# SchlomoFeng/GDN

Measured on AMD Instinct MI355X. Metric: sliding-windows/sec forward+anomaly-score, SWaT-shape (127 sensors, W=15), higher is better.
Workload: dtype f32; 1 GPU; BASELINE configs[2]: SWaT-shape eval forward + anomaly score; sensors=127, window=15, topk=30, dim=64, out_layer_num=1, batch=512, batches_per_launch=64, windows_per_launch=32768, storage=fp32, multi_gpu_measured=False, hip_graph=True, forward_streams=3, parallelism=single GPU

## Files before the change

### gdn_amd/csrc/gdn_score.hip

```cpp
#pragma clang fp contract(off)
#include "gdn_common.hpp"

#include <stdlib.h>

namespace {

constexpr int NQ = 6;

struct SelectArgs {
  int rank[NQ];
  double gamma[2];
  int median_pair;
};

constexpr unsigned long long FILLER = ~0ull;

__global__ __launch_bounds__(256) void score_keys_kernel(const float* __restrict__ pred,
                                                         const float* __restrict__ gt, int t, int n, int pitch,
                                                         double* __restrict__ keys) {
  __shared__ double tile[64][65];
  const int t0 = blockIdx.x * 64, s0 = blockIdx.y * 64;
  const int lane = threadIdx.x & 63, wv = threadIdx.x >> 6;
  for (int r = wv; r < 64; r += 4) {
    const int tick = t0 + r, s = s0 + lane;
    if (tick < t && s < n) {
      const size_t o = (size_t)tick * n + s;
      tile[r][lane] = fabs((double)pred[o] - (double)gt[o]);
    }
  }
  __syncthreads();
  for (int r = wv; r < 64; r += 4) {
    const int s = s0 + r, tick = t0 + lane;
    if (s < n && tick < pitch)
      keys[(size_t)s * pitch + tick] = tick < t ? tile[lane][r] : __longlong_as_double((long long)FILLER);
  }
}

constexpr int SLICE = 2048;

struct SelState {
  unsigned long long prefix[NQ];
  int rem[NQ];
  int rep[NQ];
  unsigned int hist[NQ][256];
  unsigned int arrive;
  unsigned int cnt_b;
  unsigned int digits_done;
  unsigned int pad1;
};

struct KeyLayout {
  const unsigned long long* keys;
  unsigned long long* bufb;
  int blocks, n, pitch;
};

__global__ void select_init_kernel(SelState* __restrict__ state, const SelectArgs sa) {
  SelState& st = state[blockIdx.x];
  for (int i = threadIdx.x; i < NQ * 256; i += blockDim.x) (&st.hist[0][0])[i] = 0u;
  if (threadIdx.x < NQ) {
    st.prefix[threadIdx.x] = 0ull;
    st.rem[threadIdx.x] = sa.rank[threadIdx.x];
    st.rep[threadIdx.x] = 0;
  }
  if (threadIdx.x == 0) {
    st.arrive = 0u;
    st.cnt_b = 0u;
    st.digits_done = 0u;
  }
}

__device__ __forceinline__ void locate_bin(const unsigned int* h, int left0, unsigned long long pf, int shift,
                                           int lane, unsigned long long* npf, int* nrem) {
  const uint4 c4 = *reinterpret_cast<const uint4*>(h + 4 * lane);
  const int mine = (int)(c4.x + c4.y + c4.z + c4.w);
  int incl = mine;
#pragma unroll
  for (int d = 1; d < 64; d <<= 1) {
    const int up = __shfl_up(incl, d);
    if (lane >= d) incl += up;
  }
  const int excl = incl - mine;
  if (left0 >= excl && left0 < incl) {
    int left = left0 - excl, bin = 0;
    const int c[4] = {(int)c4.x, (int)c4.y, (int)c4.z, (int)c4.w};
#pragma unroll
    for (int j = 0; j < 3; ++j) {
      if (bin == j && left >= c[j]) {
        left -= c[j];
        bin = j + 1;
      }
    }
    *npf = pf | ((unsigned long long)(4 * lane + bin) << shift);
    *nrem = left;
  }
}

__device__ __forceinline__ void write_result(const unsigned long long* prefix, const SelectArgs& sa, int s,
                                             double* __restrict__ med_iqr) {
  double v[NQ];
  for (int q = 0; q < NQ; ++q) v[q] = __longlong_as_double((long long)prefix[q]);
  const double med = sa.median_pair ? (v[0] + v[1]) / 2.0 : v[0];
  double qv[2];
  for (int h = 0; h < 2; ++h) {
    const double a = v[2 + 2 * h], b = v[3 + 2 * h], gm = sa.gamma[h];
    const double diff = b - a;
    double r = a + diff * gm;
    if (gm >= 0.5) r = b - diff * (1.0 - gm);
    qv[h] = r;
  }
  med_iqr[2 * s] = med;
  med_iqr[2 * s + 1] = qv[1] - qv[0];
}

template <bool FROM_B, bool COMPACT>
__global__ __launch_bounds__(256) void select_pass_kernel(const KeyLayout kl, SelState* __restrict__ state,
                                                          int pass) {
  __shared__ unsigned int hist[NQ][256];
  __shared__ unsigned long long stage[COMPACT ? SLICE : 1];
  __shared__ unsigned int n_stage, out_base, ticket_s;
  __shared__ unsigned long long npf[NQ];
  __shared__ int nrem[NQ];
  const int s = blockIdx.y, g = blockIdx.x, G = gridDim.x;
  const int tid = threadIdx.x, lane = tid & 63, wv = tid >> 6;
  SelState& st = state[s];
  if (!FROM_B && !COMPACT && pass == 1 && st.digits_done >= 2u) return;
  const unsigned int slots = (unsigned int)kl.blocks * (unsigned int)kl.pitch;
  const unsigned int cnt = FROM_B ? st.cnt_b : slots;
  unsigned long long* outb = kl.bufb + (size_t)s * slots;
  const int shift = 56 - 8 * pass;
  const bool two = !FROM_B && !COMPACT && pass == 0;
  const unsigned int dref = two ? (unsigned int)(kl.keys[(size_t)s * kl.pitch] >> 56) : 0u;
  unsigned long long pf[NQ];
  bool active[NQ];
#pragma unroll
  for (int q = 0; q < NQ; ++q) {
    pf[q] = st.prefix[q];
    active[q] = st.rep[q] == q;
  }
  for (int i = tid; i < NQ * 256; i += 256) (&hist[0][0])[i] = 0u;
  if (tid == 0) n_stage = 0u;
  __syncthreads();

  for (unsigned int base = (unsigned int)g * SLICE; base < cnt; base += (unsigned int)G * SLICE) {
    const unsigned long long* in;
    unsigned int lim;
    if (FROM_B) {
      in = outb + base;
      lim = cnt - base;
    } else {
      const unsigned int blk = base / (unsigned int)kl.pitch, off = base - blk * (unsigned int)kl.pitch;
      in = kl.keys + ((size_t)blk * kl.n + s) * kl.pitch + off;
      lim = (unsigned int)kl.pitch - off;
    }
    unsigned long long key[8];
#pragma unroll
    for (int u = 0; u < 8; ++u) {
      const unsigned int i = tid + u * 256;
      key[u] = i < lim ? in[i] : FILLER;
    }
#pragma unroll
    for (int u = 0; u < 8; ++u) {
      const bool real = key[u] != FILLER;
      const unsigned int digit = (unsigned int)(key[u] >> shift) & 255u;
      const unsigned int d0 = __builtin_amdgcn_readfirstlane(digit);
      bool any = false;
#pragma unroll
      for (int q = 0; q < NQ; ++q) {
        if (!active[q]) continue;
        const bool match = real && (pass == 0 ? true : ((key[u] ^ pf[q]) >> (shift + 8)) == 0ull);
        any |= match;
        if (__all(match && digit == d0)) {
          if (lane == 0) atomicAdd(&hist[q][d0], 64u);
        } else if (match) {
          atomicAdd(&hist[q][digit], 1u);
        }
      }
      if constexpr (COMPACT) {
        if (any) stage[atomicAdd(&n_stage, 1u)] = key[u];
      }
      if (two && real && digit == dref) atomicAdd(&hist[1][(unsigned int)(key[u] >> 48) & 255u], 1u);
    }
    if constexpr (COMPACT) {
      __syncthreads();
      if (tid == 0) out_base = n_stage ? atomicAdd(&st.cnt_b, n_stage) : 0u;
      __syncthreads();
      for (unsigned int i = tid; i < n_stage; i += 256) outb[out_base + i] = stage[i];
      __syncthreads();
      if (tid == 0) n_stage = 0u;
      __syncthreads();
    }
  }
  __syncthreads();
  for (int i = tid; i < NQ * 256; i += 256) {
    const unsigned int c = (&hist[0][0])[i];
    if (c) atomicAdd(&(&st.hist[0][0])[i], c);
  }
  asm volatile("s_waitcnt vmcnt(0)" ::: "memory");
  __syncthreads();
  if (tid == 0) ticket_s = atomicAdd(&st.arrive, 1u);
  __syncthreads();
  if (ticket_s != (unsigned int)(G - 1)) return;

  for (int i = tid; i < NQ * 256; i += 256) (&hist[0][0])[i] = atomicExch(&(&st.hist[0][0])[i], 0u);
  __syncthreads();
  for (int q = wv; q < NQ; q += 4) locate_bin(hist[st.rep[q]], st.rem[q], pf[q], shift, lane, &npf[q], &nrem[q]);
  __syncthreads();
  unsigned int done = (unsigned int)pass + 1u;
  if (two) {
    bool inside = dref != 255u;
    for (int q = 0; q < NQ; ++q) inside = inside && (unsigned int)(npf[q] >> 56) == dref;
    if (inside) {
      __shared__ unsigned long long npf2[NQ];
      __shared__ int nrem2[NQ];
      for (int q = wv; q < NQ; q += 4) locate_bin(hist[1], nrem[q], npf[q], shift - 8, lane, &npf2[q], &nrem2[q]);
      __syncthreads();
      if (tid < NQ) {
        npf[tid] = npf2[tid];
        nrem[tid] = nrem2[tid];
      }
      __syncthreads();
      done = 2u;
    }
  }
  if (tid < NQ) {
    st.prefix[tid] = npf[tid];
    st.rem[tid] = nrem[tid];
    int r = tid;
    for (int q = tid - 1; q >= 0; --q)
      if (npf[q] == npf[tid]) r = q;
    st.rep[tid] = r;
  }
  if (tid == 0) {
    st.digits_done = done;
    atomicExch(&st.arrive, 0u);
  }
}

constexpr int FIN_NT = 1024;
template <bool FROM_B>
__global__ __launch_bounds__(FIN_NT) void select_finish_kernel(const KeyLayout kl, SelState* __restrict__ state,
                                                            int first_pass, const SelectArgs sa,
                                                            double* __restrict__ med_iqr) {
  __shared__ unsigned int hist[NQ][256];
  __shared__ unsigned long long prefix[NQ];
  __shared__ int rem[NQ];
  __shared__ int rep[NQ];
  const int s = blockIdx.x;
  const int tid = threadIdx.x, lane = tid & 63, wv = tid >> 6;
  SelState& st = state[s];
  const unsigned int slots = (unsigned int)kl.blocks * (unsigned int)kl.pitch;
  const unsigned int cnt = FROM_B ? st.cnt_b : slots;
  const unsigned long long* in = FROM_B ? kl.bufb + (size_t)s * slots : kl.keys + (size_t)s * kl.pitch;
  if (tid < NQ) {
    prefix[tid] = st.prefix[tid];
    rem[tid] = st.rem[tid];
  }
  constexpr int FK = 32;
  const bool resident = cnt <= FK * FIN_NT;
  unsigned long long key[FK];
  if (resident) {
#pragma unroll
    for (int u = 0; u < FK; ++u) {
      const unsigned int i = tid + u * FIN_NT;
      key[u] = i < cnt ? in[i] : FILLER;
    }
  }
  __syncthreads();
  for (int pass = first_pass; pass < 8; ++pass) {
    const int shift = 56 - 8 * pass;
    if (tid < NQ) {
      int r = tid;
      for (int q = tid - 1; q >= 0; --q)
        if (prefix[q] == prefix[tid]) r = q;
      rep[tid] = r;
    }
    for (int i = tid; i < NQ * 256; i += FIN_NT) (&hist[0][0])[i] = 0u;
    __syncthreads();
    unsigned long long pf[NQ];
    bool active[NQ];
#pragma unroll
    for (int q = 0; q < NQ; ++q) {
      pf[q] = prefix[q];
      active[q] = rep[q] == q;
    }
    auto tally = [&](unsigned long long k) -> bool {
      if (k == FILLER) return false;
      const unsigned int digit = (unsigned int)(k >> shift) & 255u;
      bool any = false;
#pragma unroll
      for (int q = 0; q < NQ; ++q) {
        if (!active[q]) continue;
        if (pass == 0 || ((k ^ pf[q]) >> (shift + 8)) == 0ull) {
          atomicAdd(&hist[q][digit], 1u);
          any = true;
        }
      }
      return any;
    };
    if (resident) {
#pragma unroll
      for (int u = 0; u < FK; ++u)
        if (!tally(key[u])) key[u] = FILLER;
    } else {
      for (unsigned int i = tid; i < cnt; i += FIN_NT) tally(in[i]);
    }
    __syncthreads();
    for (int q = wv; q < NQ; q += FIN_NT / 64) locate_bin(hist[rep[q]], rem[q], pf[q], shift, lane, &prefix[q], &rem[q]);
    __syncthreads();
  }
  if (tid == 0) write_result(prefix, sa, s, med_iqr);
}

constexpr int ONE_NT = 1024;
constexpr int ONE_FK = 32;
constexpr int ONE_CAP = 8192;
constexpr int ONE_CAP2 = 1024;

template <bool FLAT>
__global__ __launch_bounds__(ONE_NT) void select_onewg_kernel(const KeyLayout kl, const SelectArgs sa,
                                                              double* __restrict__ med_iqr) {
  __shared__ unsigned int hist[NQ][256];
  __shared__ unsigned long long prefix[NQ];
  __shared__ unsigned long long stage[ONE_CAP];
  __shared__ unsigned long long stage2[ONE_CAP2];
  __shared__ unsigned short sidx[ONE_CAP];
  __shared__ int rem[NQ];
  __shared__ int rep[NQ];
  __shared__ unsigned int n_stage, n_stage2, dref;
  __shared__ unsigned int cnt0[2];
  const int s = blockIdx.x;
  const int tid = threadIdx.x, lane = tid & 63, wv = tid >> 6;
  const unsigned int slots = (unsigned int)kl.blocks * (unsigned int)kl.pitch;
#ifdef GDN_SELECT_TIMING
  const long long tick_start = wall_clock64();
#endif
  constexpr bool flat = FLAT;
  const __amdgpu_buffer_rsrc_t rsrc = __builtin_amdgcn_make_buffer_rsrc(
      const_cast<unsigned long long*>(kl.keys + (size_t)s * kl.pitch), 0, flat ? kl.pitch * 8 : 0, 0x00020000);
  auto key_full = [&](int u) -> unsigned long long {
    if constexpr (flat) {
      typedef unsigned int u32x2 __attribute__((ext_vector_type(2)));
      const u32x2 v = __builtin_amdgcn_raw_buffer_load_b64(rsrc, tid * 8, u * (ONE_NT * 8), 0);
      return ((unsigned long long)v.y << 32) | v.x;
    } else {
      const unsigned int i = tid + u * ONE_NT;
      const unsigned int blk = i / (unsigned int)kl.pitch, off = i - blk * (unsigned int)kl.pitch;
      return kl.keys[((size_t)blk * kl.n + s) * kl.pitch + off];
    }
  };
  auto key_slot = [&](unsigned int i) -> unsigned long long {
    if constexpr (flat) {
      return kl.keys[(size_t)s * kl.pitch + i];
    } else {
      const unsigned int blk = i / (unsigned int)kl.pitch, off = i - blk * (unsigned int)kl.pitch;
      return kl.keys[((size_t)blk * kl.n + s) * kl.pitch + off];
    }
  };
  unsigned int khi[ONE_FK];
#pragma unroll
  for (int u = 0; u < ONE_FK; ++u) {
    unsigned int hi;
    if constexpr (flat) hi = __builtin_amdgcn_raw_buffer_load_b32(rsrc, tid * 8 + 4, u * (ONE_NT * 8), 0);
    else hi = tid + u * ONE_NT < slots ? (unsigned int)(key_full(u) >> 32) : 0u;
    khi[u] = tid + u * ONE_NT < slots ? hi : 0xffffffffu;
  }
  if (tid < NQ) {
    prefix[tid] = 0ull;
    rem[tid] = sa.rank[tid];
  }
  if (tid == 0) {
    n_stage = 0u;
    n_stage2 = 0u;
  }
  __syncthreads();
#ifdef GDN_SELECT_TIMING
  long long tick[12];
  int nt = 0;
  tick[nt++] = wall_clock64();
#endif
  bool in_lds = false;
  bool done = false;
  unsigned int n_keep = 0u;
  for (int pass = 0; pass < 8 && !done; ++pass) {
    const int shift = 56 - 8 * pass;
    if (tid < NQ) {
      int r = tid;
      for (int q = tid - 1; q >= 0; --q)
        if (prefix[q] == prefix[tid]) r = q;
      rep[tid] = r;
    }
    for (int i = tid; i < NQ * 256; i += ONE_NT) (&hist[0][0])[i] = 0u;
    if (pass == 0 && tid == 0) {
      cnt0[0] = cnt0[1] = 0u;
      dref = khi[0] >> 24;
    }
    __syncthreads();
    if (pass == 0) {
      const unsigned int dr = dref;
      unsigned int less = 0u, same = 0u;
#pragma unroll
      for (int u = 0; u < ONE_FK; ++u) {
        const unsigned int hi = khi[u];
        const unsigned int digit = hi >> 24;
        less += digit < dr ? 1u : 0u;
        same += digit == dr ? 1u : 0u;
      }
#pragma unroll
      for (int d = 32; d >= 1; d >>= 1) {
        less += __shfl_xor(less, d);
        same += __shfl_xor(same, d);
      }
      if (lane == 0) {
        atomicAdd(&cnt0[0], less);
        atomicAdd(&cnt0[1], same);
      }
      __syncthreads();
      const unsigned int tl = cnt0[0], ts = cnt0[1];
      bool inside = dr != 255u;
#pragma unroll
      for (int q = 0; q < NQ; ++q) inside = inside && (unsigned int)sa.rank[q] >= tl && (unsigned int)sa.rank[q] < tl + ts;
      if (inside) {
        if (tid < NQ) {
          prefix[tid] = (unsigned long long)dr << 56;
          rem[tid] = sa.rank[tid] - (int)tl;
        }
        __syncthreads();
#ifdef GDN_SELECT_TIMING
        tick[nt++] = wall_clock64();
#endif
        continue;
      }
    }
    if (!in_lds && pass < 3) {
      const unsigned int sh = 24u - 8u * (unsigned int)pass;
#pragma nounroll
      for (int q = 0; q < NQ; ++q) {
        if (rep[q] != q) continue;
        const unsigned int pfh = (unsigned int)(prefix[q] >> 32);
        unsigned int* hq = hist[q];
#pragma unroll
        for (int u = 0; u < ONE_FK; ++u) {
          const unsigned int hi = khi[u];
          const bool real = (int)hi >= 0;
          const unsigned int digit = (hi >> sh) & 255u;
          if (pass == 0) {
            const unsigned int d0 = __builtin_amdgcn_readfirstlane(digit);
            if (__all(real && digit == d0)) {
              if (lane == 0) atomicAdd(&hq[d0], 64u);
            } else if (real) {
              atomicAdd(&hq[digit], 1u);
            }
          } else if (real && ((hi ^ pfh) >> (sh + 8u)) == 0u) {
            atomicAdd(&hq[digit], 1u);
          }
        }
      }
    } else if (!in_lds) {
#pragma nounroll
      for (int q = 0; q < NQ; ++q) {
        if (rep[q] != q) continue;
        const unsigned long long pfq = prefix[q];
        unsigned int* hq = hist[q];
#pragma unroll 4
        for (int u = 0; u < ONE_FK; ++u) {
          const bool real = (int)khi[u] >= 0;
          const unsigned long long k = real ? key_full(u) : FILLER;
          const unsigned int digit = (unsigned int)(k >> shift) & 255u;
          if (real && ((k ^ pfq) >> (shift + 8)) == 0ull) atomicAdd(&hq[digit], 1u);
        }
      }
    } else {
#pragma nounroll
      for (int q = 0; q < NQ; ++q) {
        if (rep[q] != q) continue;
        const unsigned long long pfq = prefix[q];
        unsigned int* hq = hist[q];
        for (unsigned int i = tid; i < n_keep; i += ONE_NT) {
          const unsigned long long k = stage[i];
          const unsigned int digit = (unsigned int)(k >> shift) & 255u;
          if (((k ^ pfq) >> (shift + 8)) == 0ull) atomicAdd(&hq[digit], 1u);
        }
      }
    }
    __syncthreads();
    for (int q = wv; q < NQ; q += ONE_NT / 64)
      locate_bin(hist[rep[q]], rem[q], prefix[q], shift, lane, &prefix[q], &rem[q]);
    __syncthreads();
    if (pass == 1) {
      unsigned int p16[NQ];
#pragma unroll
      for (int q = 0; q < NQ; ++q) {
        p16[q] = __builtin_amdgcn_readfirstlane((unsigned int)(prefix[q] >> 48));
#pragma unroll
        for (int r = 0; r < q; ++r)
          if (p16[r] == p16[q]) p16[q] = 0x10000u;
      }
      unsigned int keep = 0u;
#pragma unroll
      for (int u = 0; u < ONE_FK; ++u) {
        const unsigned int h16 = khi[u] >> 16;
        bool any = false;
#pragma unroll
        for (int q = 0; q < NQ; ++q) any |= h16 == p16[q];
        keep |= any ? (1u << u) : 0u;
      }
      const int mine = __popc(keep);
      int incl = mine;
#pragma unroll
      for (int d = 1; d < 64; d <<= 1) {
        const int up = __shfl_up(incl, d);
        if (lane >= d) incl += up;
      }
      unsigned int base = 0u;
      if (lane == 63) base = atomicAdd(&n_stage, (unsigned int)incl);
      base = __shfl(base, 63);
      unsigned int pos = base + (unsigned int)(incl - mine);
      unsigned int t1 = tid;
      asm volatile("" : "+v"(t1));
#pragma unroll
      for (int u = 0; u < ONE_FK; ++u) {
        if ((keep >> u) & 1u) {
          if (pos < (unsigned int)ONE_CAP) sidx[pos] = (unsigned short)(t1 + u * ONE_NT);
          ++pos;
        }
      }
      __syncthreads();
      n_keep = n_stage;
      in_lds = n_keep <= (unsigned int)ONE_CAP;
      if (in_lds) {
        for (unsigned int i = tid; i < n_keep; i += ONE_NT) stage[i] = key_slot(sidx[i]);
        __syncthreads();
      }
    }
    if (pass == 2 && in_lds) {
      for (unsigned int i = tid; i < n_keep; i += ONE_NT) {
        const unsigned long long k = stage[i];
        bool any = false;
#pragma unroll
        for (int q = 0; q < NQ; ++q) any |= ((k ^ prefix[q]) >> 40) == 0ull;
        if (any) {
          const unsigned int at = atomicAdd(&n_stage2, 1u);
          if (at < (unsigned int)ONE_CAP2) stage2[at] = k;
        }
      }
      __syncthreads();
      const unsigned int n2 = n_stage2;
      if (n2 <= (unsigned int)ONE_CAP2) {
        if ((unsigned int)tid < n2) {
          const unsigned long long k = stage2[tid];
#pragma unroll
          for (int q = 0; q < NQ; ++q) {
            const unsigned long long pq = prefix[q];
            if (((k ^ pq) >> 40) != 0ull) continue;
            int less = 0, equal = 0;
            for (unsigned int j = 0; j < n2; ++j) {
              const unsigned long long o = stage2[j];
              if (((o ^ pq) >> 40) != 0ull) continue;
              less += o < k ? 1 : 0;
              equal += o == k ? 1 : 0;
            }
            const int want = rem[q];
            if (less <= want && want < less + equal) prefix[q] = k;
          }
        }
        __syncthreads();
        done = true;
      }
    }
#ifdef GDN_SELECT_TIMING
    tick[nt++] = wall_clock64();
#endif
  }
#ifdef GDN_SELECT_TIMING
  if (tid == 0 && s == 1)
    printf("onewg ticks(10ns): load %lld p0 %lld p1+compact %lld p2+finish %lld (passes run %d) survivors %u / %u\n",
           tick[0] - tick_start, tick[1] - tick[0], tick[2] - tick[1], tick[3] - tick[2], nt - 1, n_keep, n_stage2);
#endif
  if (tid == 0) write_result(prefix, sa, s, med_iqr);
}

constexpr int RUN = 8;

__global__ __launch_bounds__(256) void score_smooth_max_kernel(
    const float* __restrict__ pred, const float* __restrict__ gt, const double* __restrict__ med_iqr,
    int t, int n, int first_tick, const float* __restrict__ halo_pred, const float* __restrict__ halo_gt,
    double* __restrict__ scores, double* __restrict__ anomaly) {
  __shared__ double best[4][RUN];
  const int lane = threadIdx.x & 63, wv = threadIdx.x >> 6;
  const int wpb = blockDim.x >> 6;
  const int nruns = (t + RUN - 1) / RUN;
  for (int run = blockIdx.x * wpb + wv; run < nruns; run += gridDim.x * wpb) {
    const int t0 = run * RUN, t1 = min(t, t0 + RUN);
    for (int s0 = 0; s0 < n; s0 += 128) {
      const int sa_ = s0 + lane, sb_ = s0 + 64 + lane;
      const bool la = sa_ < n, lb = sb_ < n;
      const int ca = la ? sa_ : n - 1, cb = lb ? sb_ : n - 1;
      const double meda = med_iqr[2 * ca], dena = 1.0 / (fabs(med_iqr[2 * ca + 1]) + 1e-2);
      const double medb = med_iqr[2 * cb], denb = 1.0 / (fabs(med_iqr[2 * cb + 1]) + 1e-2);
      const int g0 = first_tick + t0;
      float pa[RUN + 3], ga[RUN + 3], pb[RUN + 3], gb[RUN + 3];
#pragma unroll
      for (int u = 0; u < RUN + 3; ++u) {
        const int tt = t0 - 3 + u;
        const bool halo = tt < 0;
        const int row = halo ? (first_tick > 0 ? 3 + tt : 0) : min(tt, t - 1);
        const float* pp = (halo && first_tick > 0 ? halo_pred : pred) + (size_t)row * n;
        const float* gg = (halo && first_tick > 0 ? halo_gt : gt) + (size_t)row * n;
        pa[u] = pp[ca]; ga[u] = gg[ca]; pb[u] = pp[cb]; gb[u] = gg[cb];
      }
      auto norm = [&](float pv, float gv, double med, double inv_den) -> double {
        return (fabs((double)pv - (double)gv) - med) * inv_den;
      };
      double a3 = g0 >= 3 ? norm(pa[0], ga[0], meda, dena) : 0.0;
      double a2 = g0 >= 2 ? norm(pa[1], ga[1], meda, dena) : 0.0;
      double a1 = g0 >= 1 ? norm(pa[2], ga[2], meda, dena) : 0.0;
      double b3 = g0 >= 3 ? norm(pb[0], gb[0], medb, denb) : 0.0;
      double b2 = g0 >= 2 ? norm(pb[1], gb[1], medb, denb) : 0.0;
      double b1 = g0 >= 1 ? norm(pb[2], gb[2], medb, denb) : 0.0;
      double mt[RUN];
#pragma unroll
      for (int u = 0; u < RUN; ++u) {
        const int tick = t0 + u;
        mt[u] = -INFINITY;
        if (tick < t1) {
          const double a0 = norm(pa[3 + u], ga[3 + u], meda, dena);
          const double b0 = norm(pb[3 + u], gb[3 + u], medb, denb);
          double sma = 0.0, smb = 0.0;
          if (first_tick + tick >= 3) {
            sma = (((a3 + a2) + a1) + a0) / 4.0;
            smb = (((b3 + b2) + b1) + b0) / 4.0;
          }
          if (scores) {
            if (la) scores[(size_t)sa_ * t + tick] = sma;
            if (lb) scores[(size_t)sb_ * t + tick] = smb;
          }
          mt[u] = fmax(la ? sma : -INFINITY, lb ? smb : -INFINITY);
          a3 = a2; a2 = a1; a1 = a0;
          b3 = b2; b2 = b1; b1 = b0;
        }
      }
      static_assert(RUN == 8, "the transposing reduction is written for 8 ticks");
      double k4[4], k2[2], k1;
      {
        const bool up = (lane & 32) != 0;
#pragma unroll
        for (int i2 = 0; i2 < 4; ++i2) {
          const double mine = up ? mt[4 + i2] : mt[i2], send = up ? mt[i2] : mt[4 + i2];
          k4[i2] = fmax(mine, __shfl_xor(send, 32));
        }
      }
      {
        const bool up = (lane & 16) != 0;
#pragma unroll
        for (int i2 = 0; i2 < 2; ++i2) {
          const double mine = up ? k4[2 + i2] : k4[i2], send = up ? k4[i2] : k4[2 + i2];
          k2[i2] = fmax(mine, __shfl_xor(send, 16));
        }
      }
      {
        const bool up = (lane & 8) != 0;
        const double mine = up ? k2[1] : k2[0], send = up ? k2[0] : k2[1];
        k1 = fmax(mine, __shfl_xor(send, 8));
      }
      k1 = fmax(k1, __shfl_xor(k1, 4));
      k1 = fmax(k1, __shfl_xor(k1, 2));
      k1 = fmax(k1, __shfl_xor(k1, 1));
      if ((lane & 7) == 0) {
        const int u = ((lane >> 5) & 1) * 4 + ((lane >> 4) & 1) * 2 + ((lane >> 3) & 1);
        best[wv][u] = s0 == 0 ? k1 : fmax(best[wv][u], k1);
      }
    }
    if (lane < t1 - t0) anomaly[t0 + lane] = best[wv][lane];
  }
}

}

namespace {

SelectArgs make_select_args(long long t) {
  SelectArgs sa;
  sa.median_pair = (t % 2 == 0);
  sa.rank[0] = (int)(sa.median_pair ? t / 2 - 1 : (t - 1) / 2);
  sa.rank[1] = (int)(sa.median_pair ? t / 2 : (t - 1) / 2);
  const double qs[2] = {25.0 / 100.0, 75.0 / 100.0};
  for (int h = 0; h < 2; ++h) {
    const double vi = (double)t * qs[h] + (1.0 + qs[h] * (1.0 - 1.0 - 1.0)) - 1.0;
    const double lo = floor(vi);
    long long ilo = (long long)lo, ihi = ilo + 1;
    if (ilo < 0) ilo = 0;
    if (ihi > t - 1) ihi = t - 1;
    if (ilo > t - 1) ilo = t - 1;
    sa.rank[2 + 2 * h] = (int)ilo;
    sa.rank[3 + 2 * h] = (int)ihi;
    sa.gamma[h] = vi - lo;
  }
  return sa;
}

bool force_multi_block() {
  static int v = -1;
  if (v < 0) {
    const char* e = getenv("GDN_SELECT_MULTI");
    v = (e && e[0] == '1') ? 1 : 0;
  }
  return v == 1;
}

int run_select(const double* keys, int blocks, int n, int pitch, long long total, double* workspace,
               double* med_iqr, hipStream_t st) {
  const long long slots = (long long)blocks * pitch;
  KeyLayout kl;
  kl.keys = reinterpret_cast<const unsigned long long*>(keys);
  kl.bufb = reinterpret_cast<unsigned long long*>(workspace);
  kl.blocks = blocks; kl.n = n; kl.pitch = pitch;
  SelState* state = reinterpret_cast<SelState*>(kl.bufb + (size_t)slots * n);
  const SelectArgs sa = make_select_args(total);
  const int slices = (int)((slots + SLICE - 1) / SLICE);
  if (slices > 1 && slots <= (long long)ONE_NT * ONE_FK && !force_multi_block()) {
    if (kl.blocks == 1) hipLaunchKernelGGL(select_onewg_kernel<true>, dim3(n), dim3(ONE_NT), 0, st, kl, sa, med_iqr);
    else hipLaunchKernelGGL(select_onewg_kernel<false>, dim3(n), dim3(ONE_NT), 0, st, kl, sa, med_iqr);
    return gdn_launch_status();
  }
  hipLaunchKernelGGL(select_init_kernel, dim3(n), dim3(256), 0, st, state, sa);
  if (slices == 1) {
    hipLaunchKernelGGL(select_finish_kernel<false>, dim3(n), dim3(FIN_NT), 0, st, kl, state, 0, sa, med_iqr);
    return gdn_launch_status();
  }
  hipLaunchKernelGGL((select_pass_kernel<false, false>), dim3(slices, n), dim3(256), 0, st, kl, state, 0);
  hipLaunchKernelGGL((select_pass_kernel<false, false>), dim3(slices, n), dim3(256), 0, st, kl, state, 1);
  hipLaunchKernelGGL((select_pass_kernel<false, true>), dim3(slices, n), dim3(256), 0, st, kl, state, 2);
  hipLaunchKernelGGL(select_finish_kernel<true>, dim3(n), dim3(FIN_NT), 0, st, kl, state, 3, sa, med_iqr);
  return gdn_launch_status();
}

}

extern "C" long long gdn_score_select_workspace_bytes(int blocks, int n, int pitch) {
  if (blocks <= 0 || n <= 0 || pitch <= 0) return 0;
  return (long long)blocks * pitch * n * 8 + (long long)n * (long long)sizeof(SelState) + 256;
}

extern "C" long long gdn_score_workspace_bytes(int t, int n) {
  if (t <= 0 || n <= 0) return 0;
  return (long long)t * n * 8 + gdn_score_select_workspace_bytes(1, n, t);
}

extern "C" int gdn_score_keys(const float* pred, const float* gt, int t, int n, int pitch, double* keys,
                              void* stream) {
  if (!pred || !gt || !keys || t <= 0 || n <= 0 || pitch < t) return GDN_ERR_ARG;
  hipLaunchKernelGGL(score_keys_kernel, dim3((pitch + 63) / 64, (n + 63) / 64), dim3(256), 0,
                     (hipStream_t)stream, pred, gt, t, n, pitch, keys);
  return gdn_launch_status();
}

extern "C" int gdn_score_select(const double* keys, int blocks, int n, int pitch, long long total,
                                double* workspace, double* med_iqr, void* stream) {
  if (!keys || !workspace || !med_iqr || blocks <= 0 || n <= 0 || pitch <= 0 || total <= 0) return GDN_ERR_ARG;
  if (total > (long long)blocks * pitch || (long long)blocks * pitch > 0x7fffffffll) return GDN_ERR_ARG;
  if (blocks > 1 && pitch % SLICE != 0) return GDN_ERR_UNSUPPORTED;
  return run_select(keys, blocks, n, pitch, total, workspace, med_iqr, (hipStream_t)stream);
}

extern "C" int gdn_score_quantiles(const float* pred, const float* gt, int t, int n, double* workspace,
                                   double* med_iqr, void* stream) {
  if (!pred || !gt || !workspace || !med_iqr || t <= 0 || n <= 0) return GDN_ERR_ARG;
  double* keys = workspace;
  const int rc = gdn_score_keys(pred, gt, t, n, t, keys, stream);
  if (rc != GDN_OK) return rc;
  return run_select(keys, 1, n, t, t, workspace + (size_t)t * n, med_iqr, (hipStream_t)stream);
}

extern "C" int gdn_score_smooth_max(const float* pred, const float* gt, const double* med_iqr, int t, int n,
                                    int first_tick, const float* halo_pred, const float* halo_gt,
                                    double* scores, double* anomaly, void* stream) {
  if (!pred || !gt || !med_iqr || !anomaly || t <= 0 || n <= 0 || first_tick < 0) return GDN_ERR_ARG;
  if (first_tick > 0 && (!halo_pred || !halo_gt)) return GDN_ERR_ARG;
  const int runs = (t + RUN - 1) / RUN;
  const int grid = min((runs + 3) / 4, gdn_cu_count() * 8);
  hipLaunchKernelGGL(score_smooth_max_kernel, dim3(grid), dim3(256), 0, (hipStream_t)stream, pred, gt,
                     med_iqr, t, n, first_tick, halo_pred, halo_gt, scores, anomaly);
  return gdn_launch_status();
}
```

Baseline: 137.7 million windows/s.

## Select quantiles from a compact 32-bit high-word plane, recomputing low bits on demand

```diff
diff --git a/gdn_amd/csrc/gdn_score.hip b/gdn_amd/csrc/gdn_score.hip
--- a/gdn_amd/csrc/gdn_score.hip
+++ b/gdn_amd/csrc/gdn_score.hip
@@ -14,25 +14,31 @@
 };
 
 constexpr unsigned long long FILLER = ~0ull;
-
+constexpr unsigned int FILLER_HI = ~0u;
+
+__device__ __forceinline__ unsigned long long score_key(const float* __restrict__ pred, const float* __restrict__ gt,
+                                                        size_t o) {
+  return (unsigned long long)__double_as_longlong(fabs((double)pred[o] - (double)gt[o]));
+}
+
+template <typename K>
 __global__ __launch_bounds__(256) void score_keys_kernel(const float* __restrict__ pred,
                                                          const float* __restrict__ gt, int t, int n, int pitch,
-                                                         double* __restrict__ keys) {
-  __shared__ double tile[64][65];
+                                                         K* __restrict__ keys) {
+  __shared__ K tile[64][65];
   const int t0 = blockIdx.x * 64, s0 = blockIdx.y * 64;
   const int lane = threadIdx.x & 63, wv = threadIdx.x >> 6;
   for (int r = wv; r < 64; r += 4) {
     const int tick = t0 + r, s = s0 + lane;
     if (tick < t && s < n) {
-      const size_t o = (size_t)tick * n + s;
-      tile[r][lane] = fabs((double)pred[o] - (double)gt[o]);
+      const unsigned long long key = score_key(pred, gt, (size_t)tick * n + s);
+      tile[r][lane] = sizeof(K) == 8 ? (K)key : (K)(key >> 32);
     }
   }
   __syncthreads();
   for (int r = wv; r < 64; r += 4) {
     const int s = s0 + r, tick = t0 + lane;
-    if (s < n && tick < pitch)
-      keys[(size_t)s * pitch + tick] = tick < t ? tile[lane][r] : __longlong_as_double((long long)FILLER);
+    if (s < n && tick < pitch) keys[(size_t)s * pitch + tick] = tick < t ? tile[lane][r] : (K)FILLER;
   }
 }
 
@@ -580,6 +586,237 @@
   if (tid == 0) write_result(prefix, sa, s, med_iqr);
 }
 
+constexpr unsigned int NO_PREFIX = 0x80000000u;
+
+__global__ __launch_bounds__(ONE_NT) void select_onewg_hi_kernel(const unsigned int* __restrict__ plane, int pitch,
+                                                                 const float* __restrict__ pred,
+                                                                 const float* __restrict__ gt, int n,
+                                                                 const SelectArgs sa, double* __restrict__ med_iqr) {
+  __shared__ unsigned int hist[NQ][256];
+  __shared__ unsigned long long prefix[NQ];
+  __shared__ unsigned long long cand[ONE_CAP];
+  __shared__ int rem[NQ];
+  __shared__ int rep[NQ];
+  __shared__ unsigned int n_cand, dref;
+  __shared__ unsigned int cnt0[2];
+  const int s = blockIdx.x;
+  const int tid = threadIdx.x, lane = tid & 63, wv = tid >> 6;
+  const unsigned int slots = (unsigned int)pitch;
+#ifdef GDN_SELECT_TIMING
+  const long long tick_start = wall_clock64();
+#endif
+  const __amdgpu_buffer_rsrc_t rsrc = __builtin_amdgcn_make_buffer_rsrc(
+      const_cast<unsigned int*>(plane + (size_t)s * pitch), 0, pitch * 4, 0x00020000);
+  unsigned int khi[ONE_FK];
+#pragma unroll
+  for (int u = 0; u < ONE_FK; ++u) {
+    const unsigned int hi = __builtin_amdgcn_raw_buffer_load_b32(rsrc, tid * 4, u * (ONE_NT * 4), 0);
+    khi[u] = tid + u * ONE_NT < slots ? hi : FILLER_HI;
+  }
+  if (tid < NQ) {
+    prefix[tid] = 0ull;
+    rem[tid] = sa.rank[tid];
+  }
+  if (tid == 0) n_cand = 0u;
+  __syncthreads();
+#ifdef GDN_SELECT_TIMING
+  long long tick[12];
+  int nt = 0;
+  tick[nt++] = wall_clock64();
+#endif
+  bool in_lds = false;
+  unsigned int n_keep = 0u;
+  for (int pass = 0; pass < 8; ++pass) {
+    const int shift = 56 - 8 * pass;
+    if (tid < NQ) {
+      int r = tid;
+      for (int q = tid - 1; q >= 0; --q)
+        if (prefix[q] == prefix[tid]) r = q;
+      rep[tid] = r;
+    }
+    for (int i = tid; i < NQ * 256; i += ONE_NT) (&hist[0][0])[i] = 0u;
+    if (pass == 0 && tid == 0) {
+      cnt0[0] = cnt0[1] = 0u;
+      dref = khi[0] >> 24;
+    }
+    __syncthreads();
+    if (pass == 0) {
+      const unsigned int dr = dref;
+      unsigned int less = 0u, same = 0u;
+#pragma unroll
+      for (int u = 0; u < ONE_FK; ++u) {
+        const unsigned int digit = khi[u] >> 24;
+        less += digit < dr ? 1u : 0u;
+        same += digit == dr ? 1u : 0u;
+      }
+#pragma unroll
+      for (int d = 32; d >= 1; d >>= 1) {
+        less += __shfl_xor(less, d);
+        same += __shfl_xor(same, d);
+      }
+      if (lane == 0) {
+        atomicAdd(&cnt0[0], less);
+        atomicAdd(&cnt0[1], same);
+      }
+      __syncthreads();
+      const unsigned int tl = cnt0[0], ts = cnt0[1];
+      bool inside = dr != 255u;
+#pragma unroll
+      for (int q = 0; q < NQ; ++q) inside = inside && (unsigned int)sa.rank[q] >= tl && (unsigned int)sa.rank[q] < tl + ts;
+      if (inside) {
+        if (tid < NQ) {
+          prefix[tid] = (unsigned long long)dr << 56;
+          rem[tid] = sa.rank[tid] - (int)tl;
+        }
+        __syncthreads();
+#ifdef GDN_SELECT_TIMING
+        tick[nt++] = wall_clock64();
+#endif
+        continue;
+      }
+    }
+    if (pass < 4) {
+      const unsigned int sh = 24u - 8u * (unsigned int)pass;
+#pragma nounroll
+      for (int q = 0; q < NQ; ++q) {
+        if (rep[q] != q) continue;
+        const unsigned int pfh = (unsigned int)(prefix[q] >> 32);
+        unsigned int* hq = hist[q];
+#pragma unroll
+        for (int u = 0; u < ONE_FK; ++u) {
+          const unsigned int hi = khi[u];
+          const bool real = (int)hi >= 0;
+          const unsigned int digit = (hi >> sh) & 255u;
+          if (pass == 0) {
+            const unsigned int d0 = __builtin_amdgcn_readfirstlane(digit);
+            if (__all(real && digit == d0)) {
+              if (lane == 0) atomicAdd(&hq[d0], 64u);
+            } else if (real) {
+              atomicAdd(&hq[digit], 1u);
+            }
+          } else if (real && ((hi ^ pfh) >> (sh + 8u)) == 0u) {
+            atomicAdd(&hq[digit], 1u);
+          }
+        }
+      }
+    } else if (in_lds) {
+#pragma nounroll
+      for (int q = 0; q < NQ; ++q) {
+        if (rep[q] != q) continue;
+        const unsigned long long pfq = prefix[q];
+        unsigned int* hq = hist[q];
+        for (unsigned int i = tid; i < n_keep; i += ONE_NT) {
+          const unsigned long long k = cand[i];
+          const unsigned int digit = (unsigned int)(k >> shift) & 255u;
+          if (((k ^ pfq) >> (shift + 8)) == 0ull) atomicAdd(&hq[digit], 1u);
+        }
+      }
+    } else {
+#pragma nounroll
+      for (int q = 0; q < NQ; ++q) {
+        if (rep[q] != q) continue;
+        const unsigned long long pfq = prefix[q];
+        const unsigned int pfh = (unsigned int)(pfq >> 32);
+        unsigned int* hq = hist[q];
+        unsigned int t1 = tid;
+        asm volatile("" : "+v"(t1));
+#pragma unroll
+        for (int u = 0; u < ONE_FK; ++u) {
+          if (khi[u] != pfh) continue;
+          const unsigned long long k = score_key(pred, gt, (size_t)(t1 + u * ONE_NT) * n + s);
+          const unsigned int digit = (unsigned int)(k >> shift) & 255u;
+          if (((k ^ pfq) >> (shift + 8)) == 0ull) atomicAdd(&hq[digit], 1u);
+        }
+      }
+    }
+    __syncthreads();
+    for (int q = wv; q < NQ; q += ONE_NT / 64)
+      locate_bin(hist[rep[q]], rem[q], prefix[q], shift, lane, &prefix[q], &rem[q]);
+    __syncthreads();
+#ifdef GDN_SELECT_TIMING
+    if (pass < 3) tick[nt++] = wall_clock64();
+#endif
+    if (pass == 3) {
+      unsigned int ph[NQ], p32[NQ];
+#pragma unroll
+      for (int q = 0; q < NQ; ++q) {
+        ph[q] = __builtin_amdgcn_readfirstlane((unsigned int)(prefix[q] >> 32));
+        p32[q] = ph[q];
+#pragma unroll
+        for (int r = 0; r < q; ++r)
+          if (ph[r] == ph[q]) p32[q] = NO_PREFIX;
+      }
+      unsigned int keep = 0u;
+#pragma unroll
+      for (int u = 0; u < ONE_FK; ++u) {
+        bool any = false;
+#pragma unroll
+        for (int q = 0; q < NQ; ++q) any |= khi[u] == p32[q];
+        keep |= any ? (1u << u) : 0u;
+      }
+      if (__any(keep != 0u)) {
+        const int mine = __popc(keep);
+        int incl = mine;
+#pragma unroll
+        for (int d = 1; d < 64; d <<= 1) {
+          const int up = __shfl_up(incl, d);
+          if (lane >= d) incl += up;
+        }
+        unsigned int base = 0u;
+        if (lane == 63) base = atomicAdd(&n_cand, (unsigned int)incl);
+        base = __shfl(base, 63);
+        unsigned int pos = base + (unsigned int)(incl - mine);
+        unsigned int t1 = tid;
+        asm volatile("" : "+v"(t1));
+#pragma unroll
+        for (int u = 0; u < ONE_FK; ++u) {
+          if ((keep >> u) & 1u) {
+            if (pos < (unsigned int)ONE_CAP) cand[pos] = (unsigned long long)(t1 + u * ONE_NT);
+            ++pos;
+          }
+        }
+      }
+      __syncthreads();
+      n_keep = n_cand;
+      in_lds = n_keep <= (unsigned int)ONE_CAP;
+      if (in_lds) {
+        for (unsigned int i = tid; i < n_keep; i += ONE_NT) cand[i] = score_key(pred, gt, (size_t)cand[i] * n + s);
+        __syncthreads();
+        if (n_keep <= (unsigned int)ONE_CAP2) {
+          if ((unsigned int)tid < n_keep) {
+            const unsigned long long k = cand[tid];
+            const unsigned int kh = (unsigned int)(k >> 32);
+            int less = 0, equal = 0;
+            for (unsigned int j = 0; j < n_keep; ++j) {
+              const unsigned long long o = cand[j];
+              if ((unsigned int)(o >> 32) != kh) continue;
+              less += o < k ? 1 : 0;
+              equal += o == k ? 1 : 0;
+            }
+#pragma unroll
+            for (int q = 0; q < NQ; ++q) {
+              const int want = rem[q];
+              if (kh == ph[q] && less <= want && want < less + equal) prefix[q] = k;
+            }
+          }
+          __syncthreads();
+#ifdef GDN_SELECT_TIMING
+          tick[nt++] = wall_clock64();
+#endif
+          break;
+        }
+      }
+    }
+  }
+#ifdef GDN_SELECT_TIMING
+  while (nt < 5) tick[nt++] = wall_clock64();
+  if (tid == 0 && s == 1)
+    printf("onewg-hi ticks(10ns): load %lld p0 %lld p1 %lld p2 %lld p3+finish %lld survivors %u\n",
+           tick[0] - tick_start, tick[1] - tick[0], tick[2] - tick[1], tick[3] - tick[2], tick[4] - tick[3], n_keep);
+#endif
+  if (tid == 0) write_result(prefix, sa, s, med_iqr);
+}
+
 constexpr int RUN = 8;
 
 __global__ __launch_bounds__(256) void score_smooth_max_kernel(
@@ -708,6 +945,19 @@
   return v == 1;
 }
 
+bool compact_plane_enabled() {
+  static int v = -1;
+  if (v < 0) {
+    const char* e = getenv("GDN_SCORE_COMPACT");
+    v = (e && e[0] == '0') ? 0 : 1;
+  }
+  return v == 1;
+}
+
+bool one_workgroup_size(long long slots) {
+  return slots > SLICE && slots <= (long long)ONE_NT * ONE_FK && !force_multi_block();
+}
+
 int run_select(const double* keys, int blocks, int n, int pitch, long long total, double* workspace,
                double* med_iqr, hipStream_t st) {
   const long long slots = (long long)blocks * pitch;
@@ -718,7 +968,7 @@
   SelState* state = reinterpret_cast<SelState*>(kl.bufb + (size_t)slots * n);
   const SelectArgs sa = make_select_args(total);
   const int slices = (int)((slots + SLICE - 1) / SLICE);
-  if (slices > 1 && slots <= (long long)ONE_NT * ONE_FK && !force_multi_block()) {
+  if (one_workgroup_size(slots)) {
     if (kl.blocks == 1) hipLaunchKernelGGL(select_onewg_kernel<true>, dim3(n), dim3(ONE_NT), 0, st, kl, sa, med_iqr);
     else hipLaunchKernelGGL(select_onewg_kernel<false>, dim3(n), dim3(ONE_NT), 0, st, kl, sa, med_iqr);
     return gdn_launch_status();
@@ -750,8 +1000,8 @@
 extern "C" int gdn_score_keys(const float* pred, const float* gt, int t, int n, int pitch, double* keys,
                               void* stream) {
   if (!pred || !gt || !keys || t <= 0 || n <= 0 || pitch < t) return GDN_ERR_ARG;
-  hipLaunchKernelGGL(score_keys_kernel, dim3((pitch + 63) / 64, (n + 63) / 64), dim3(256), 0,
-                     (hipStream_t)stream, pred, gt, t, n, pitch, keys);
+  hipLaunchKernelGGL(score_keys_kernel<unsigned long long>, dim3((pitch + 63) / 64, (n + 63) / 64), dim3(256), 0,
+                     (hipStream_t)stream, pred, gt, t, n, pitch, reinterpret_cast<unsigned long long*>(keys));
   return gdn_launch_status();
 }
 
@@ -766,6 +1016,14 @@
 extern "C" int gdn_score_quantiles(const float* pred, const float* gt, int t, int n, double* workspace,
                                    double* med_iqr, void* stream) {
   if (!pred || !gt || !workspace || !med_iqr || t <= 0 || n <= 0) return GDN_ERR_ARG;
+  if (one_workgroup_size(t) && compact_plane_enabled()) {
+    unsigned int* plane = reinterpret_cast<unsigned int*>(workspace);
+    hipLaunchKernelGGL(score_keys_kernel<unsigned int>, dim3((t + 63) / 64, (n + 63) / 64), dim3(256), 0,
+                       (hipStream_t)stream, pred, gt, t, n, t, plane);
+    hipLaunchKernelGGL(select_onewg_hi_kernel, dim3(n), dim3(ONE_NT), 0, (hipStream_t)stream, plane, t, pred, gt, n,
+                       make_select_args(t), med_iqr);
+    return gdn_launch_status();
+  }
   double* keys = workspace;
   const int rc = gdn_score_keys(pred, gt, t, n, t, keys, stream);
   if (rc != GDN_OK) return rc;
```

After: 129.3 million windows/s. -6.1%, worse.
